# googlegenomics/spark-examples

Measured on NVIDIA H100. Metric: genotype-cells/sec (N x V) into Gram, higher is better.
Workload: dtype int8

## Files before the change

### spark_examples_b200/csrc/gram_sm90.cu

```cuda
#include <cuda.h>
#include <cuda_runtime.h>

#include <cstring>

#include <algorithm>
#include <map>
#include <mutex>
#include <tuple>
#include <type_traits>
#include <cstdio>
#include <cstdlib>
#include <string>
#include <vector>

#include "ptx_sm90.cuh"
#include "vpca_internal.h"

namespace vpca {

namespace {

constexpr int kThreads = 384;
constexpr int kKBytes = 128;
constexpr int kBoxRows = 128;
// ... 22 lines not shown
    int flags;
    int acc_cols;
    int pad1;
};
constexpr int kTileXpose = 1, kTileFiller = 2, kTileSelfB = 4;
constexpr int kMaxSegs = 4;

struct GramArgs {
    int32_t* S;
    int32_t* peer[kMaxPeers];
    int num_peers;
    int peer_mode;
    int own_end[kMaxPeers];
    const TileDesc* tiles;
    int* err;
    int n;
    int num_tiles;
    int num_full;
    int total_weight;
    int kb_total;
    int kb_window;
    int num_workers;
    int resident;
    int kc_per_kb;
    int kb_per_panel;
    int sync_lead;
    int active_workers;
    int* win_done;
    long long* prof;
    const double* cum;
    int col_limit;
    int acc_stride;
    int row_limit;
    int red64;
};

struct Seg {
    int tile, kb0, kb1, col, slot, first, flush, use, win, last_in_win;
    int rowA0, rowA1, rowB, n_eff, flags;
};

struct SegPlan {
    int n;
    int tile[kMaxSegs], lo[kMaxSegs], hi[kMaxSegs], col[kMaxSegs];
    int cols;
    int overflow;
};

__host__ __device__ inline void plan_segments(const TileDesc* tiles, int num_tiles, int first_tile, long long u_begin,
                                              long long u_end, int len, SegPlan& p) {
    p.n = 0;
    p.cols = 0;
    p.overflow = 0;
    const long long origin = (long long)tiles[first_tile].wstart * len;
    long long u = u_begin;
    int t = first_tile;
    while (u < u_end && t < num_tiles) {
        const int w = tiles[t].n_eff >> 4;
        const long long base = (long long)tiles[t].wstart * len - origin;
        const long long tend = base + (long long)w * len;
        if (tend <= u) {
            ++t;
            continue;
        }
        const long long e = u_end < tend ? u_end : tend;
        const int lo = (int)((u - base) / w);
        const int hi = e == tend ? len : (int)((e - base) / w);
// ... 222 lines not shown
        __nanosleep(256);
    }
}

__device__ __forceinline__ uint64_t make_smem_desc(uint32_t saddr) {
    return (uint64_t)((saddr & 0x3FFFFu) >> 4) | (1ull << 16) | ((uint64_t)(1024 >> 4) << 32) | (1ull << 62);
}

__device__ __forceinline__ uint32_t e2m1x4_to_s8x2(uint32_t w) {
    const uint32_t mag = __byte_perm(0x03020100u, 0x0C080604u, w & 0x7777u);
    const uint32_t sgn = ((w >> 3) & 1u) | (((w >> 7) & 1u) << 8) | (((w >> 11) & 1u) << 16) | (((w >> 15) & 1u) << 24);
    const uint32_t m = sgn * 0xFFu;
    return (mag & ~m) | (__vneg4(mag) & m);
}

__device__ __forceinline__ int quarter_rn(int acc) {
    const int q = acc >> 2, r = acc & 3;
    return q + ((r > 2 || (r == 2 && (q & 1))) ? 1 : 0);
}

template <int KIND>
using AccT = typename std::conditional<KIND == 1, float, uint32_t>::type;

template <int KIND>
__device__ __forceinline__ int acc_to_int(AccT<KIND> v) {
    if constexpr (KIND == 0) return (int)v;
    else if constexpr (KIND == 1) return __float2int_rn(v);
    else return quarter_rn((int)v);
}

template <int CG, int KIND>
__global__ void __launch_bounds__(kThreads, 1) gram_kernel(const __grid_constant__ CUtensorMap tmap, const GramArgs a) {
    using C = Cfg<KIND>;
    extern __shared__ uint8_t smem_raw[];
    const uint32_t smem_base = (ptx::smem_u32(smem_raw) + 1023u) & ~1023u;
    const uint32_t bar_base = smem_base + C::STAGES * C::STAGE_BYTES + C::XBUF_BYTES * 2;
    auto sB = [&](uint32_t st) { return smem_base + st * C::STAGE_BYTES; };
    auto sA = [&](uint32_t st) { return smem_base + st * C::STAGE_BYTES + C::B_BYTES; };
    auto full_bar = [&](uint32_t i) { return bar_base + 8u * i; };
    auto empty_bar = [&](uint32_t i) { return bar_base + 8u * (C::STAGES + i); };

    const int warp = __shfl_sync(0xffffffffu, (int)(threadIdx.x >> 5), 0);
    const uint32_t lane = ptx::lane_id();
    const uint32_t cta_rank = (CG == 2) ? (blockIdx.x & 1u) : 0u;
    const int worker = (CG == 2) ? (int)(blockIdx.x >> 1) : (int)blockIdx.x;
    auto release = [&](uint32_t st) {
        if constexpr (CG == 2) {
            ptx::mbar_arrive_cluster(ptx::mapa(empty_bar(st), 0));
            ptx::mbar_arrive_cluster(ptx::mapa(empty_bar(st), 1));
        } else {
            ptx::mbar_arrive(empty_bar(st));
        }
    };

    if (warp == 0 && ptx::elect_one()) {
        ptx::prefetch_tensormap(&tmap);
        for (uint32_t i = 0; i < (uint32_t)C::STAGES; ++i) {
            ptx::mbar_init(full_bar(i), 1);
            ptx::mbar_init(empty_bar(i), 2 * CG);
        }
        ptx::fence_mbar_init();
    }
    if constexpr (CG == 2) ptx::cluster_sync();
    else __syncthreads();
    if (a.prof != nullptr && threadIdx.x == 0) a.prof[(size_t)blockIdx.x * 4 + 0] = globaltimer_ns();

    if (warp < 4) {
        asm volatile("setmaxnreg.dec.sync.aligned.u32 40;");
        if (warp == 0 && ptx::elect_one()) {
            const bool leader = cta_rank == 0;
            Sched sc;
            sc.init(a, worker);
            Seg s;
            uint32_t it = 0;
            int synced_win = -1;
            while (sc.next(s)) {
                const int rowA = (CG == 2 && cta_rank != 0) ? s.rowA1 : s.rowA0;
                const bool two_boxes = s.n_eff > kBoxRows;
                const bool self_b = (CG == 2) && (s.flags & kTileSelfB) != 0;
                const uint32_t tx = (uint32_t)((two_boxes ? 2 : 1) + (self_b ? 0 : 1)) * C::BOX_BYTES;
                if (a.sync_lead > 0 && leader && s.win != synced_win) {
                    synced_win = s.win;
                    if (s.win >= a.sync_lead) wait_window(a.win_done, s.win - a.sync_lead, a.active_workers);
                }
                for (int kb = s.kb0; kb < s.kb1; ++kb, ++it) {
                    const uint32_t st = it % C::STAGES, ph = (it / C::STAGES) & 1u;
                    mbar_wait(empty_bar(st), ph ^ 1u, a.err, 1);
                    const int pnl = kb / a.kb_per_panel;
                    const int kc = (kb - pnl * a.kb_per_panel) * a.kc_per_kb;
                    ptx::mbar_arrive_expect_tx(full_bar(st), tx);
                    if constexpr (CG == 2) {
                        if (two_boxes || cta_rank == 0)
                            ptx::tma_load_3d_multicast(sB(st) + cta_rank * C::BOX_BYTES, &tmap, full_bar(st), kc,
                                                       s.rowB + (int)cta_rank * kBoxRows, pnl, 0x3);
                    } else {
                        ptx::tma_load_3d(sB(st), &tmap, full_bar(st), kc, s.rowB, pnl);
                        if (two_boxes) ptx::tma_load_3d(sB(st) + C::BOX_BYTES, &tmap, full_bar(st), kc, s.rowB + kBoxRows, pnl);
                    }
                    if (!self_b) ptx::tma_load_3d(sA(st), &tmap, full_bar(st), kc, rowA, pnl);
                }
                if (a.sync_lead > 0 && leader && s.last_in_win)
                    asm volatile("red.release.gpu.global.add.s32 [%0], 1;" ::"l"(a.win_done + s.win) : "memory");
            }
        }
    } else {
        asm volatile("setmaxnreg.inc.sync.aligned.u32 232;");
        const int cw = (warp >> 2) - 1;
        const int wq = warp & 3;
        const uint32_t ctid = threadIdx.x - 128;
        AccT<KIND> acc[2][64];
        Sched sc;
        sc.init(a, worker);
        Seg s;
        uint32_t it = 0;
        while (sc.next(s)) {
            const bool filler = (CG == 2) && cta_rank != 0 && (s.flags & kTileFiller) != 0;
            const bool self_b = (CG == 2) && (s.flags & kTileSelfB) != 0;
            const int mrow0 = cw * 128;
            const bool act0 = mrow0 < s.n_eff, act1 = mrow0 + 64 < s.n_eff;
            if (s.first) {
#pragma unroll
                for (int i = 0; i < 64; ++i) {
                    acc[0][i] = 0;
                    acc[1][i] = 0;
                }
            }
            const uint32_t a_off = (self_b ? cta_rank : 2u) * (uint32_t)(kBoxRows * 128);
            int pending = -1;
            for (int kb = s.kb0; kb < s.kb1; ++kb, ++it) {
                const uint32_t st = it % C::STAGES, ph = (it / C::STAGES) & 1u;
                mbar_wait(full_bar(st), ph, a.err, 3);
                uint32_t opB, opA;
                if constexpr (KIND == 2) {
                    const uint32_t xb = smem_base + C::STAGES * C::STAGE_BYTES + (it & 1u) * C::XBUF_BYTES;
                    ptx::named_sync(1, 256);
                    const int nb = s.n_eff > kBoxRows ? 2 * kBoxRows : kBoxRows;
                    const int rows = nb + (self_b ? 0 : kBoxRows);
                    for (int c = (int)ctid; c < rows * 8; c += 256) {
                        const int r = c >> 3, j = c & 7;
                        const uint32_t src = (r < nb ? sB(st) + (uint32_t)r * 64u : sA(st) + (uint32_t)(r - nb) * 64u) + (uint32_t)j * 8u;
                        const int xr = r < nb ? r : 2 * kBoxRows + (r - nb);
                        uint32_t lo, hi;
                        asm volatile("ld.shared.v2.u32 {%0, %1}, [%2];" : "=r"(lo), "=r"(hi) : "r"(src));
                        const uint32_t o0 = e2m1x4_to_s8x2(lo & 0xFFFFu), o1 = e2m1x4_to_s8x2(lo >> 16);
                        const uint32_t o2 = e2m1x4_to_s8x2(hi & 0xFFFFu), o3 = e2m1x4_to_s8x2(hi >> 16);
                        const uint32_t dst = xb + (uint32_t)xr * 128u + (((uint32_t)j ^ ((uint32_t)xr & 7u)) << 4);
                        asm volatile("st.shared.v4.u32 [%0], {%1, %2, %3, %4};" ::"r"(dst), "r"(o0), "r"(o1), "r"(o2), "r"(o3)
                                     : "memory");
                    }
                    ptx::fence_proxy_async();
                    ptx::named_sync(1, 256);
                    if (threadIdx.x % 128 == 0) release(st);
                    opB = xb;
                } else {
                    opB = sB(st);
                }
                opA = opB + a_off;
                const uint64_t bdesc = make_smem_desc(opA);
                const uint64_t adesc0 = make_smem_desc(opB + (uint32_t)mrow0 * 128u);
                const uint64_t adesc1 = make_smem_desc(opB + (uint32_t)(mrow0 + 64) * 128u);
                ptx::wgmma_fence_acc(acc[0]);
                ptx::wgmma_fence_acc(acc[1]);
                ptx::wgmma_fence();
#pragma unroll
                for (int k = 0; k < kKBytes / 32; ++k) {
                    if constexpr (KIND == 1) {
                        ptx::wgmma_bf16(acc[0], adesc0 + 2 * k, bdesc + 2 * k);
                        ptx::wgmma_bf16(acc[1], adesc1 + 2 * k, bdesc + 2 * k);
                    } else {
                        ptx::wgmma_s8(acc[0], adesc0 + 2 * k, bdesc + 2 * k);
                        ptx::wgmma_s8(acc[1], adesc1 + 2 * k, bdesc + 2 * k);
                    }
                }
                ptx::wgmma_commit();
                ptx::wgmma_wait<1>();
                ptx::wgmma_fence_acc(acc[0]);
                ptx::wgmma_fence_acc(acc[1]);
                if constexpr (KIND != 2) {
                    if (pending >= 0 && threadIdx.x % 128 == 0) release((uint32_t)pending);
                }
                pending = (int)st;
            }
            ptx::wgmma_wait<0>();
            ptx::wgmma_fence_acc(acc[0]);
            ptx::wgmma_fence_acc(acc[1]);
            if constexpr (KIND != 2) {
                if (pending >= 0 && threadIdx.x % 128 == 0) release((uint32_t)pending);
            }
            if (!s.flush || filler) continue;

            const int colA = (CG == 2 && cta_rank != 0) ? s.rowA1 : s.rowA0;
            const int row_end = min(a.row_limit, s.rowB + s.n_eff);
            const bool pair64 = a.red64 != 0 && (a.n & 1) == 0;
#pragma unroll
            for (int j = 0; j < 2; ++j) {
                if (!(j == 0 ? act0 : act1)) continue;
#pragma unroll
                for (int h = 0; h < 2; ++h) {
                    const int row = s.rowB + mrow0 + 64 * j + 16 * wq + (int)(lane >> 2) + 8 * h;
                    if (row >= row_end) continue;
                    int32_t* own = a.S;
                    if (a.num_peers != 0 && a.peer_mode == 1) {
                        int o = 0;
                        while (o + 1 < a.num_peers && row >= a.own_end[o]) ++o;
                        own = a.peer[o];
                    }
#pragma unroll
                    for (int i = 0; i < 16; ++i) {
                        const int col = colA + 8 * i + 2 * (int)(lane & 3);
                        if (col >= a.n) continue;
                        int v0 = acc_to_int<KIND>(acc[j][4 * i + 2 * h]);
                        int v1 = acc_to_int<KIND>(acc[j][4 * i + 2 * h + 1]);
                        if ((s.flags & kTileXpose) != 0 && (row >> 7) < (col >> 7)) {
                            for (int e = 0; e < 2; ++e) {
                                const int v = e ? v1 : v0, c = col + e;
                                if (v == 0 || c >= a.n) continue;
                                const size_t o = (size_t)c * (size_t)a.n + (size_t)row;
                                if (a.num_peers == 0) {
                                    asm volatile("red.global.add.s32 [%0], %1;" ::"l"(a.S + o), "r"(v) : "memory");
                                } else if (a.peer_mode == 1) {
                                    int q = 0;
                                    while (q + 1 < a.num_peers && c >= a.own_end[q]) ++q;
                                    asm volatile("red.relaxed.sys.global.add.s32 [%0], %1;" ::"l"(a.peer[q] + o), "r"(v) : "memory");
                                } else {
                                    for (int d = 0; d < a.num_peers; ++d)
                                        asm volatile("red.relaxed.sys.global.add.s32 [%0], %1;" ::"l"(a.peer[d] + o), "r"(v)
                                                     : "memory");
                                }
                            }
                            continue;
                        }
                        if (row < col) v0 = 0;
                        if (row < col + 1 || col + 1 >= a.n) v1 = 0;
                        if ((v0 | v1) == 0) continue;
                        const size_t o = (size_t)row * (size_t)a.n + (size_t)col;
                        if (pair64) {
                            const unsigned long long packed = (unsigned long long)(unsigned)v0 | ((unsigned long long)(unsigned)v1 << 32);
                            if (a.num_peers == 0) {
                                asm volatile("red.global.add.u64 [%0], %1;" ::"l"(a.S + o), "l"(packed) : "memory");
                            } else if (a.peer_mode == 1) {
                                asm volatile("red.relaxed.sys.global.add.u64 [%0], %1;" ::"l"(own + o), "l"(packed) : "memory");
                            } else {
                                for (int d = 0; d < a.num_peers; ++d)
                                    asm volatile("red.relaxed.sys.global.add.u64 [%0], %1;" ::"l"(a.peer[d] + o), "l"(packed)
                                                 : "memory");
                            }
                        } else {
                            for (int e = 0; e < 2; ++e) {
                                const int v = e ? v1 : v0;
                                if (v == 0) continue;
                                if (a.num_peers == 0) {
                                    asm volatile("red.global.add.s32 [%0], %1;" ::"l"(a.S + o + e), "r"(v) : "memory");
                                } else if (a.peer_mode == 1) {
                                    asm volatile("red.relaxed.sys.global.add.s32 [%0], %1;" ::"l"(own + o + e), "r"(v) : "memory");
                                } else {
                                    for (int d = 0; d < a.num_peers; ++d)
                                        asm volatile("red.relaxed.sys.global.add.s32 [%0], %1;" ::"l"(a.peer[d] + o + e), "r"(v)
                                                     : "memory");
                                }
                            }
                        }
                    }
                }
            }
        }
        if (a.prof != nullptr && threadIdx.x == 128) a.prof[(size_t)blockIdx.x * 4 + 2] = globaltimer_ns();
    }

    if constexpr (CG == 2) ptx::cluster_sync();
    else __syncthreads();
    if (a.prof != nullptr && threadIdx.x == 0) a.prof[(size_t)blockIdx.x * 4 + 3] = globaltimer_ns();
}

__global__ void rebalance_kernel(const long long* __restrict__ prof, double* __restrict__ cum, int workers, int cta_group,
                                 double gain, double max_share, long long min_ns, int* __restrict__ gen, const TileDesc* __restrict__ tiles,
                                 int num_tiles, int total_weight, int kbw, int col_limit) {
    __shared__ double sh[1024];
    __shared__ double cand[1025];
    __shared__ long long need[1025];
    __shared__ double red_sum, red_min;
    __shared__ int reject, need_repair;
    const int w = threadIdx.x;
    const bool active = w < workers;
    double t = 0.0, share_old = 0.0;
    if (active) {
        const long long t0 = prof[(size_t)w * cta_group * 4 + 0], t1 = prof[(size_t)w * cta_group * 4 + 2];
        t = (double)(t1 - t0);
        share_old = cum[w + 1] - cum[w];
    }
    sh[w] = active ? t : 1e30;
    if (w == 0) {
        reject = 0;
        need_repair = 0;
// ... 460 lines not shown
        for (int i = 0; i < p.n; ++i, ++cnt)
            if (cnt < max_pieces) {
                int32_t* o = out + (size_t)cnt * 6;
                o[0] = w; o[1] = p.tile[i]; o[2] = p.lo[i]; o[3] = p.hi[i]; o[4] = p.col[i]; o[5] = p.cols;
            }
    }
    return cnt;
}

cudaError_t gram_accumulate(GramPlan& plan, const void* d_x, int elem_bits, int n, int64_t nv, int64_t ld, int64_t panel,
                            int32_t* d_S, cudaStream_t stream, std::string* err) {
    if (nv <= 0) return cudaSuccess;
    EncodeTiledFn encode = get_encode_fn();
    if (encode == nullptr) {
        if (err) *err = "cuTensorMapEncodeTiled entry point not available";
        return cudaErrorNotSupported;
    }
    if (plan.num_sms == 0) {
        int dev = 0;
        cudaGetDevice(&dev);
        cudaDeviceGetAttribute(&plan.num_sms, cudaDevAttrMultiProcessorCount, dev);
        const char* cg = getenv("VPCA_CTA_GROUP");
        if (cg != nullptr) plan.cta_group = (atoi(cg) == 1) ? 1 : 2;
        const char* kw = getenv("VPCA_KB_WINDOW");
        if (kw != nullptr) plan.kb_window = atoi(kw);
        const char* sl = getenv("VPCA_SYNC_LEAD");
        if (sl != nullptr) plan.sync_lead = atoi(sl);
        const char* pf = getenv("VPCA_GRAM_PROF");
        plan.profile = (pf != nullptr && atoi(pf) != 0);
        const char* ad = getenv("VPCA_ADAPTIVE");
        if (ad != nullptr) plan.adaptive = atoi(ad) != 0;
        const char* sb = getenv("VPCA_SELF_B");
        if (sb != nullptr) plan.self_b = atoi(sb) != 0;
        const char* r64 = getenv("VPCA_RED64");
        if (r64 != nullptr) plan.red64 = atoi(r64) != 0;
        const char* gain = getenv("VPCA_REBALANCE_GAIN");
        if (gain != nullptr) plan.gain = std::min(1.0, std::max(0.1, atof(gain)));
        const char* ex = getenv("VPCA_EXACT_COVER");
        if (ex != nullptr) plan.exact_cover = atoi(ex) != 0;
    }
    if (plan.d_win_done == nullptr) {
        cudaError_t e = cudaMalloc(&plan.d_win_done, GramPlan::kMaxWindows * sizeof(int));
        if (e != cudaSuccess) return e;
    }
    if ((plan.profile || plan.adaptive) && plan.d_prof == nullptr) {
        cudaError_t e = cudaMalloc(&plan.d_prof, 1024 * 4 * sizeof(long long));
        if (e != cudaSuccess) return e;
        e = cudaMemsetAsync(plan.d_prof, 0, 1024 * 4 * sizeof(long long), stream);
        if (e != cudaSuccess) return e;
    }
    if (plan.d_err == nullptr) {
        cudaError_t e = cudaHostAlloc(&plan.d_err, 4 * sizeof(int), cudaHostAllocMapped);
        if (e != cudaSuccess) return e;
        for (int i = 0; i < 4; ++i) plan.d_err[i] = 0;
    }
    const int tile_bn = kUmmaN;
    const bool banded = plan.own_hi > plan.own_lo && plan.num_peers <= 1;
    const int row_lo = banded ? plan.own_lo : 0, row_hi = banded ? plan.own_hi : n;
    const bool exact = plan.exact_cover && !banded;
    if (plan.tiles_for_n != n || plan.tiles_for_cg != plan.cta_group || plan.tiles_for_bn != (exact ? -1 : tile_bn) ||
        plan.tiles_row_lo != row_lo || plan.tiles_row_hi != row_hi) {
        cudaError_t e = build_tiles(plan, n, exact, tile_bn, row_lo, row_hi, stream);
        if (e != cudaSuccess) return e;
    }
    if (panel > 0) {
        if ((panel % 128) != 0) {
            if (err) *err = "panel_variants must be a multiple of 128";
            return cudaErrorInvalidValue;
// ... 30 lines not shown
                                   (cuuint64_t)n * (cuuint64_t)ld * (cuuint64_t)elem_bits / 8};
    const int kc_per_kb = elem_bits == 4 ? elems_per_kb / 2 : elems_per_kb;
    const cuuint32_t box[3] = {(cuuint32_t)kc_per_kb, (cuuint32_t)kBoxRows, 1};
    const cuuint32_t estr[3] = {1, 1, 1};
    const CUtensorMapDataType tmtype = elem_bits == 16 ? CU_TENSOR_MAP_DATA_TYPE_BFLOAT16 : CU_TENSOR_MAP_DATA_TYPE_UINT8;
    CUresult r = encode(&tmap, tmtype, 3,
                        const_cast<void*>(d_x), gdim, gstride, box, estr, CU_TENSOR_MAP_INTERLEAVE_NONE,
                        elem_bits == 4 ? CU_TENSOR_MAP_SWIZZLE_NONE : CU_TENSOR_MAP_SWIZZLE_128B,
                        CU_TENSOR_MAP_L2_PROMOTION_L2_256B, CU_TENSOR_MAP_FLOAT_OOB_FILL_NONE);
    if (r != CUDA_SUCCESS) {
        if (err) *err = "cuTensorMapEncodeTiled failed with CUresult " + std::to_string((int)r);
        return cudaErrorInvalidValue;
    }

    GramArgs args{};
    args.S = banded ? d_S - (ptrdiff_t)plan.own_lo * n : d_S;
    args.num_peers = (plan.num_peers > 1 && d_S == plan.peer_base[plan.peer_rank]) ? plan.num_peers : 0;
    for (int d = 0; d < kMaxPeers; ++d) args.peer[d] = d < plan.num_peers ? plan.peer_S[d] : nullptr;
    args.peer_mode = plan.peer_mode;
    for (int d = 0; d < kMaxPeers; ++d) args.own_end[d] = plan.own_end[d];
    args.tiles = static_cast<const TileDesc*>(plan.d_tiles);
    cudaHostGetDevicePointer(reinterpret_cast<void**>(&args.err), plan.d_err, 0);
    args.n = n;
    args.num_tiles = plan.num_tiles;
    args.num_full = plan.num_full;
    args.total_weight = plan.total_weight;
    args.kb_total = (int)((nv + elems_per_kb - 1) / elems_per_kb);
    args.kb_per_panel = panel > 0 ? (int)(panel / elems_per_kb) : args.kb_total;
    args.num_workers = workers;
    args.kc_per_kb = kc_per_kb;
    args.acc_stride = 0;
    args.col_limit = plan.tiles_col_limit;
    args.row_limit = row_hi;
    args.red64 = plan.red64 ? 1 : 0;
    {
        int kbw = plan.kb_window;
        if (kbw <= 0 && panel > 0) kbw = args.kb_per_panel;
        if (kbw <= 0) {
            const long long target = 16ll << 20;
            kbw = (int)std::max<long long>(8, std::min<long long>(4096, target / ((long long)n * kKBytes)));
        }
        kbw = std::min(kbw, args.kb_total);
        std::vector<double> cum0;
        args.resident = (plan.num_tiles <= 4 * workers && initial_split(plan, workers, kbw, cum0)) ? 1 : 0;
        int dev = 0;
        cudaGetDevice(&dev);
        args.kb_window = args.resident ? kbw : args.kb_total;
        if (args.resident && (plan.d_cum == nullptr || plan.cum_workers != workers || plan.cum_tiles != plan.num_tiles ||
                              plan.cum_kbw != kbw || plan.cum_for_n != n || plan.cum_elem != elem_bits)) {
            remember_split(plan);
            if (plan.adaptive && !banded) {
                std::lock_guard<std::mutex> lk(g_split_mu);
                auto it = g_splits.find(SplitKey{dev, n, plan.num_tiles, kbw, workers, elem_bits});
                if (it != g_splits.end()) {
                    std::vector<double> learned = it->second;
                    const TileDesc* tiles = reinterpret_cast<const TileDesc*>(plan.h_tiles.data());
                    std::vector<long long> need((size_t)workers + 1);
                    if (repair_split(tiles, plan.num_tiles, workers, (long long)plan.total_weight * kbw, kbw, plan.tiles_col_limit,
                                     learned.data(), need.data()))
                        cum0 = learned;
                }
            }
            if (plan.d_cum) cudaFree(plan.d_cum);
            plan.d_cum = nullptr;
            cudaError_t e = cudaMalloc(&plan.d_cum, (size_t)(workers + 2) * sizeof(double) + sizeof(int));
            if (e != cudaSuccess) return e;
            cum0.push_back(0.0);
// ... 128 lines not shown
```

### spark_examples_b200/csrc/ptx_sm90.cuh

```cuda
#pragma once
#include <cstdint>
#include <cuda_runtime.h>

namespace vpca {
namespace ptx {

__device__ __forceinline__ uint32_t smem_u32(const void* p) {
    return static_cast<uint32_t>(__cvta_generic_to_shared(p));
}

__device__ __forceinline__ uint32_t lane_id() {
    uint32_t r;
    asm volatile("mov.u32 %0, %%laneid;" : "=r"(r));
    return r;
}

__device__ __forceinline__ bool elect_one() {
    uint32_t pred = 0;
    asm volatile(
        "{\n\t"
        ".reg .pred P;\n\t"
        "elect.sync _|P, 0xffffffff;\n\t"
        "selp.u32 %0, 1, 0, P;\n\t"
        "}\n"
// ... 60 lines not shown
    asm volatile("barrier.cluster.arrive.release;\n\tbarrier.cluster.wait.acquire;" ::: "memory");
}
__device__ __forceinline__ void wgmma_fence() { asm volatile("wgmma.fence.sync.aligned;" ::: "memory"); }
__device__ __forceinline__ void wgmma_commit() { asm volatile("wgmma.commit_group.sync.aligned;" ::: "memory"); }
template <int N>
__device__ __forceinline__ void wgmma_wait() { asm volatile("wgmma.wait_group.sync.aligned %0;" ::"n"(N) : "memory"); }
__device__ __forceinline__ void wgmma_fence_acc(uint32_t (&d)[64]) {
#pragma unroll
    for (int i = 0; i < 64; ++i) asm volatile("" : "+r"(d[i])::"memory");
}
__device__ __forceinline__ void wgmma_fence_acc(float (&d)[64]) {
#pragma unroll
    for (int i = 0; i < 64; ++i) asm volatile("" : "+f"(d[i])::"memory");
}

__device__ __forceinline__ void wgmma_s8(uint32_t (&d)[64], uint64_t a_desc, uint64_t b_desc) {
    asm volatile(
        "{\n\t.reg .pred p;\n\tsetp.ne.b32 p, 1, 0;\n\t"
        "wgmma.mma_async.sync.aligned.m64n128k32.s32.s8.s8 "
        "{%0, %1, %2, %3, %4, %5, %6, %7, %8, %9, %10, %11, %12, %13, %14, %15, %16, %17, %18, %19, %20, %21, %22, %23, %24, %25, %26, %27, %28, %29, %30, %31, %32, %33, %34, %35, %36, %37, %38, %39, %40, %41, %42, %43, %44, %45, %46, %47, %48, %49, %50, %51, %52, %53, %54, %55, %56, %57, %58, %59, %60, %61, %62, %63}, %64, %65, p;\n\t}\n"
        : "+r"(d[0]), "+r"(d[1]), "+r"(d[2]), "+r"(d[3]), "+r"(d[4]), "+r"(d[5]), "+r"(d[6]), "+r"(d[7]), "+r"(d[8]), "+r"(d[9]), "+r"(d[10]), "+r"(d[11]), "+r"(d[12]), "+r"(d[13]), "+r"(d[14]), "+r"(d[15]), "+r"(d[16]), "+r"(d[17]), "+r"(d[18]), "+r"(d[19]), "+r"(d[20]), "+r"(d[21]), "+r"(d[22]), "+r"(d[23]), "+r"(d[24]), "+r"(d[25]), "+r"(d[26]), "+r"(d[27]), "+r"(d[28]), "+r"(d[29]), "+r"(d[30]), "+r"(d[31]), "+r"(d[32]), "+r"(d[33]), "+r"(d[34]), "+r"(d[35]), "+r"(d[36]), "+r"(d[37]), "+r"(d[38]), "+r"(d[39]), "+r"(d[40]), "+r"(d[41]), "+r"(d[42]), "+r"(d[43]), "+r"(d[44]), "+r"(d[45]), "+r"(d[46]), "+r"(d[47]), "+r"(d[48]), "+r"(d[49]), "+r"(d[50]), "+r"(d[51]), "+r"(d[52]), "+r"(d[53]), "+r"(d[54]), "+r"(d[55]), "+r"(d[56]), "+r"(d[57]), "+r"(d[58]), "+r"(d[59]), "+r"(d[60]), "+r"(d[61]), "+r"(d[62]), "+r"(d[63])
        : "l"(a_desc), "l"(b_desc));
}

__device__ __forceinline__ void wgmma_bf16(float (&f)[64], uint64_t a_desc, uint64_t b_desc) {
    asm volatile(
        "{\n\t.reg .pred p;\n\tsetp.ne.b32 p, 1, 0;\n\t"
        "wgmma.mma_async.sync.aligned.m64n128k16.f32.bf16.bf16 "
        "{%0, %1, %2, %3, %4, %5, %6, %7, %8, %9, %10, %11, %12, %13, %14, %15, %16, %17, %18, %19, %20, %21, %22, %23, %24, %25, %26, %27, %28, %29, %30, %31, %32, %33, %34, %35, %36, %37, %38, %39, %40, %41, %42, %43, %44, %45, %46, %47, %48, %49, %50, %51, %52, %53, %54, %55, %56, %57, %58, %59, %60, %61, %62, %63}, %64, %65, p, 1, 1, 0, 0;\n\t}\n"
        : "+f"(f[0]), "+f"(f[1]), "+f"(f[2]), "+f"(f[3]), "+f"(f[4]), "+f"(f[5]), "+f"(f[6]), "+f"(f[7]), "+f"(f[8]), "+f"(f[9]), "+f"(f[10]), "+f"(f[11]), "+f"(f[12]), "+f"(f[13]), "+f"(f[14]), "+f"(f[15]), "+f"(f[16]), "+f"(f[17]), "+f"(f[18]), "+f"(f[19]), "+f"(f[20]), "+f"(f[21]), "+f"(f[22]), "+f"(f[23]), "+f"(f[24]), "+f"(f[25]), "+f"(f[26]), "+f"(f[27]), "+f"(f[28]), "+f"(f[29]), "+f"(f[30]), "+f"(f[31]), "+f"(f[32]), "+f"(f[33]), "+f"(f[34]), "+f"(f[35]), "+f"(f[36]), "+f"(f[37]), "+f"(f[38]), "+f"(f[39]), "+f"(f[40]), "+f"(f[41]), "+f"(f[42]), "+f"(f[43]), "+f"(f[44]), "+f"(f[45]), "+f"(f[46]), "+f"(f[47]), "+f"(f[48]), "+f"(f[49]), "+f"(f[50]), "+f"(f[51]), "+f"(f[52]), "+f"(f[53]), "+f"(f[54]), "+f"(f[55]), "+f"(f[56]), "+f"(f[57]), "+f"(f[58]), "+f"(f[59]), "+f"(f[60]), "+f"(f[61]), "+f"(f[62]), "+f"(f[63])
        : "l"(a_desc), "l"(b_desc));
}

__device__ __forceinline__ void named_sync(uint32_t id, uint32_t count) {
    asm volatile("bar.sync %0, %1;" ::"r"(id), "r"(count) : "memory");
}

}
}
```

### spark_examples_b200/csrc/vpca_internal.h

```cpp
#pragma once
#include <cstdint>
#include <cuda_runtime.h>
#include <string>
#include <vector>

#include "../../include/vpca.h"

namespace vpca {

struct GramPlan {
    int cta_group = 2;
    int kb_window = 0;
    int num_sms = 0;
    int max_pairs[3] = {};
    void* d_tiles = nullptr;
    std::vector<int32_t> h_tiles;
    int num_tiles = 0;
    int num_full = 0;
    int total_weight = 0;
    int tiles_col_limit = 256;
    bool exact_cover = false;
    int tiles_for_n = -1;
    int tiles_for_cg = 0;
    int tiles_for_bn = 0;
    int tiles_row_lo = 0, tiles_row_hi = 0;
    int own_lo = 0, own_hi = 0;
    int last_resident = 0;
    int* d_err = nullptr;
    static constexpr int kMaxWindows = 1 << 16;
    int sync_lead = 0;
    int* d_win_done = nullptr;
    bool self_b = true;
    bool red64 = true;
    double gain = 0.5;
    bool adaptive = true;
    double* d_cum = nullptr;
    int cum_workers = 0, cum_tiles = 0, cum_kbw = 0, cum_for_n = 0, cum_dev = 0, cum_elem = 0;
    int num_peers = 0, peer_rank = 0, peer_epoch = 0;
    int32_t* peer_S[16] = {};
    int32_t* peer_base[16] = {};
    int32_t* peer_flags[16] = {};
    int band_row0[16] = {}, band_rows[16] = {};
    bool peers_ipc = false;
    int peer_mode = 0;
    int own_end[16] = {};
    bool profile = false;
    long long* d_prof = nullptr;
};
int gram_read_profile(GramPlan& plan, long long* out, int max_ctas);

cudaError_t gram_accumulate(GramPlan& plan, const void* d_x, int elem_bits, int n, int64_t nv, int64_t ld, int64_t panel,
                            int32_t* d_S, cudaStream_t stream, std::string* err);
cudaError_t gram_symmetrize(int32_t* d_S, int n, cudaStream_t stream);
cudaError_t gram_add(int32_t* d_dst, const int32_t* d_src, int64_t count, cudaStream_t stream);
cudaError_t gram_add_peers(GramPlan& plan, const int32_t* d_src, int64_t count, cudaStream_t stream);
cudaError_t gram_add_owners(GramPlan& plan, const int32_t* d_src, int n, cudaStream_t stream);
cudaError_t gram_gather_rows(GramPlan& plan, int32_t* d_S, int n, cudaStream_t stream);
cudaError_t gram_peer_barrier(GramPlan& plan, cudaStream_t stream);
cudaError_t gram_preload_kernels(cudaStream_t stream);
cudaError_t encode_preload_kernels();
void gram_plan_free(GramPlan& plan);
int gram_debug_max_clusters(int cluster_size);
int gram_debug_band_tiles(int n, int cta_group, int row_lo, int row_hi, int32_t* out, int max_tiles);
int gram_debug_tiles(int n, int cta_group, int exact, int32_t* out, int max_tiles);
int gram_debug_plan(const int32_t* tiles8, int num_tiles, int workers, int kbw, int32_t* out, int max_pieces);
int gram_debug_repair(const int32_t* tiles8, int num_tiles, int workers, int kbw, int col_limit, double* cum, int32_t* out,
// ... 152 lines not shown
```

Before: 534.4 billion.

## Use m64n256 WGMMA with multicast A tiles for 2-CTA cluster path

For the 2-CTA cluster configuration (non-FP4 kinds), each CTA now loads its own 128-row B slice and both A boxes arrive by multicast. Each consumer warpgroup then issues a single m64n256 WGMMA covering both A column blocks instead of two m64n128 instructions. Flush logic is remapped so the second accumulator writes to rowA1 columns. This halves WGMMA issue count and raises per-instruction N, improving operand reuse. The cost is a changed shared-memory layout and filler-tile handling, plus reliance on a multicast of A that must match the cluster scheduling.

```diff
diff --git a/spark_examples_b200/csrc/gram_sm90.cu b/spark_examples_b200/csrc/gram_sm90.cu
--- a/spark_examples_b200/csrc/gram_sm90.cu
+++ b/spark_examples_b200/csrc/gram_sm90.cu
@@ -367,11 +367,13 @@
 template <int CG, int KIND>
 __global__ void __launch_bounds__(kThreads, 1) gram_kernel(const __grid_constant__ CUtensorMap tmap, const GramArgs a) {
     using C = Cfg<KIND>;
+    constexpr bool WIDE = CG == 2 && KIND != 2;
+    constexpr uint32_t kBBytes = WIDE ? C::BOX_BYTES : C::B_BYTES;
     extern __shared__ uint8_t smem_raw[];
     const uint32_t smem_base = (ptx::smem_u32(smem_raw) + 1023u) & ~1023u;
     const uint32_t bar_base = smem_base + C::STAGES * C::STAGE_BYTES + C::XBUF_BYTES * 2;
     auto sB = [&](uint32_t st) { return smem_base + st * C::STAGE_BYTES; };
-    auto sA = [&](uint32_t st) { return smem_base + st * C::STAGE_BYTES + C::B_BYTES; };
+    auto sA = [&](uint32_t st) { return smem_base + st * C::STAGE_BYTES + kBBytes; };
     auto full_bar = [&](uint32_t i) { return bar_base + 8u * i; };
     auto empty_bar = [&](uint32_t i) { return bar_base + 8u * (C::STAGES + i); };
 
@@ -423,6 +425,13 @@
                     mbar_wait(empty_bar(st), ph ^ 1u, a.err, 1);
                     const int pnl = kb / a.kb_per_panel;
                     const int kc = (kb - pnl * a.kb_per_panel) * a.kc_per_kb;
+                    if constexpr (WIDE) {
+                        ptx::mbar_arrive_expect_tx(full_bar(st), (uint32_t)(self_b ? 2 : 3) * C::BOX_BYTES);
+                        if (!self_b)
+                            ptx::tma_load_3d(sB(st), &tmap, full_bar(st), kc, s.rowB + (int)cta_rank * kBoxRows, pnl);
+                        ptx::tma_load_3d_multicast(sA(st) + cta_rank * C::BOX_BYTES, &tmap, full_bar(st), kc, rowA, pnl, 0x3);
+                        continue;
+                    }
                     ptx::mbar_arrive_expect_tx(full_bar(st), tx);
                     if constexpr (CG == 2) {
                         if (two_boxes || cta_rank == 0)
@@ -449,10 +458,10 @@
         Seg s;
         uint32_t it = 0;
         while (sc.next(s)) {
-            const bool filler = (CG == 2) && cta_rank != 0 && (s.flags & kTileFiller) != 0;
+            const bool filler = (CG == 2) && (WIDE || cta_rank != 0) && (s.flags & kTileFiller) != 0;
             const bool self_b = (CG == 2) && (s.flags & kTileSelfB) != 0;
-            const int mrow0 = cw * 128;
-            const bool act0 = mrow0 < s.n_eff, act1 = mrow0 + 64 < s.n_eff;
+            const int mrow0 = WIDE ? (int)cta_rank * 128 + cw * 64 : cw * 128;
+            const bool act0 = mrow0 < s.n_eff, act1 = WIDE ? act0 && !filler : mrow0 + 64 < s.n_eff;
             if (s.first) {
 #pragma unroll
                 for (int i = 0; i < 64; ++i) {
@@ -491,15 +500,24 @@
                     opB = sB(st);
                 }
                 opA = opB + a_off;
+                if constexpr (WIDE) {
+                    opA = sA(st);
+                    opB = self_b ? opA + cta_rank * (uint32_t)C::BOX_BYTES : sB(st);
+                }
                 const uint64_t bdesc = make_smem_desc(opA);
                 const uint64_t adesc0 = make_smem_desc(opB + (uint32_t)mrow0 * 128u);
                 const uint64_t adesc1 = make_smem_desc(opB + (uint32_t)(mrow0 + 64) * 128u);
+                const uint64_t adescw = make_smem_desc(opB + (uint32_t)(cw * 64) * 128u);
                 ptx::wgmma_fence_acc(acc[0]);
                 ptx::wgmma_fence_acc(acc[1]);
                 ptx::wgmma_fence();
 #pragma unroll
                 for (int k = 0; k < kKBytes / 32; ++k) {
-                    if constexpr (KIND == 1) {
+                    if constexpr (WIDE && KIND == 1) {
+                        ptx::wgmma_bf16_n256(acc[0], acc[1], adescw + 2 * k, bdesc + 2 * k);
+                    } else if constexpr (WIDE) {
+                        ptx::wgmma_s8_n256(acc[0], acc[1], adescw + 2 * k, bdesc + 2 * k);
+                    } else if constexpr (KIND == 1) {
                         ptx::wgmma_bf16(acc[0], adesc0 + 2 * k, bdesc + 2 * k);
                         ptx::wgmma_bf16(acc[1], adesc1 + 2 * k, bdesc + 2 * k);
                     } else {
@@ -522,9 +540,9 @@
             if constexpr (KIND != 2) {
                 if (pending >= 0 && threadIdx.x % 128 == 0) release((uint32_t)pending);
             }
-            if (!s.flush || filler) continue;
-
-            const int colA = (CG == 2 && cta_rank != 0) ? s.rowA1 : s.rowA0;
+            if (!s.flush || (filler && !WIDE)) continue;
+
+            const int colA = (CG == 2 && cta_rank != 0 && !WIDE) ? s.rowA1 : s.rowA0;
             const int row_end = min(a.row_limit, s.rowB + s.n_eff);
             const bool pair64 = a.red64 != 0 && (a.n & 1) == 0;
 #pragma unroll
@@ -532,7 +550,7 @@
                 if (!(j == 0 ? act0 : act1)) continue;
 #pragma unroll
                 for (int h = 0; h < 2; ++h) {
-                    const int row = s.rowB + mrow0 + 64 * j + 16 * wq + (int)(lane >> 2) + 8 * h;
+                    const int row = s.rowB + mrow0 + (WIDE ? 0 : 64 * j) + 16 * wq + (int)(lane >> 2) + 8 * h;
                     if (row >= row_end) continue;
                     int32_t* own = a.S;
                     if (a.num_peers != 0 && a.peer_mode == 1) {
@@ -542,7 +560,7 @@
                     }
 #pragma unroll
                     for (int i = 0; i < 16; ++i) {
-                        const int col = colA + 8 * i + 2 * (int)(lane & 3);
+                        const int col = (WIDE && j == 1 ? s.rowA1 : colA) + 8 * i + 2 * (int)(lane & 3);
                         if (col >= a.n) continue;
                         int v0 = acc_to_int<KIND>(acc[j][4 * i + 2 * h]);
                         int v1 = acc_to_int<KIND>(acc[j][4 * i + 2 * h + 1]);
diff --git a/spark_examples_b200/csrc/ptx_sm90.cuh b/spark_examples_b200/csrc/ptx_sm90.cuh
--- a/spark_examples_b200/csrc/ptx_sm90.cuh
+++ b/spark_examples_b200/csrc/ptx_sm90.cuh
@@ -116,6 +116,24 @@
         : "l"(a_desc), "l"(b_desc));
 }
 
+__device__ __forceinline__ void wgmma_s8_n256(uint32_t (&d0)[64], uint32_t (&d1)[64], uint64_t a_desc, uint64_t b_desc) {
+    asm volatile(
+        "{\n\t.reg .pred p;\n\tsetp.ne.b32 p, 1, 0;\n\t"
+        "wgmma.mma_async.sync.aligned.m64n256k32.s32.s8.s8 "
+        "{%0, %1, %2, %3, %4, %5, %6, %7, %8, %9, %10, %11, %12, %13, %14, %15, %16, %17, %18, %19, %20, %21, %22, %23, %24, %25, %26, %27, %28, %29, %30, %31, %32, %33, %34, %35, %36, %37, %38, %39, %40, %41, %42, %43, %44, %45, %46, %47, %48, %49, %50, %51, %52, %53, %54, %55, %56, %57, %58, %59, %60, %61, %62, %63, %64, %65, %66, %67, %68, %69, %70, %71, %72, %73, %74, %75, %76, %77, %78, %79, %80, %81, %82, %83, %84, %85, %86, %87, %88, %89, %90, %91, %92, %93, %94, %95, %96, %97, %98, %99, %100, %101, %102, %103, %104, %105, %106, %107, %108, %109, %110, %111, %112, %113, %114, %115, %116, %117, %118, %119, %120, %121, %122, %123, %124, %125, %126, %127}, %128, %129, p;\n\t}\n"
+        : "+r"(d0[0]), "+r"(d0[1]), "+r"(d0[2]), "+r"(d0[3]), "+r"(d0[4]), "+r"(d0[5]), "+r"(d0[6]), "+r"(d0[7]), "+r"(d0[8]), "+r"(d0[9]), "+r"(d0[10]), "+r"(d0[11]), "+r"(d0[12]), "+r"(d0[13]), "+r"(d0[14]), "+r"(d0[15]), "+r"(d0[16]), "+r"(d0[17]), "+r"(d0[18]), "+r"(d0[19]), "+r"(d0[20]), "+r"(d0[21]), "+r"(d0[22]), "+r"(d0[23]), "+r"(d0[24]), "+r"(d0[25]), "+r"(d0[26]), "+r"(d0[27]), "+r"(d0[28]), "+r"(d0[29]), "+r"(d0[30]), "+r"(d0[31]), "+r"(d0[32]), "+r"(d0[33]), "+r"(d0[34]), "+r"(d0[35]), "+r"(d0[36]), "+r"(d0[37]), "+r"(d0[38]), "+r"(d0[39]), "+r"(d0[40]), "+r"(d0[41]), "+r"(d0[42]), "+r"(d0[43]), "+r"(d0[44]), "+r"(d0[45]), "+r"(d0[46]), "+r"(d0[47]), "+r"(d0[48]), "+r"(d0[49]), "+r"(d0[50]), "+r"(d0[51]), "+r"(d0[52]), "+r"(d0[53]), "+r"(d0[54]), "+r"(d0[55]), "+r"(d0[56]), "+r"(d0[57]), "+r"(d0[58]), "+r"(d0[59]), "+r"(d0[60]), "+r"(d0[61]), "+r"(d0[62]), "+r"(d0[63]), "+r"(d1[0]), "+r"(d1[1]), "+r"(d1[2]), "+r"(d1[3]), "+r"(d1[4]), "+r"(d1[5]), "+r"(d1[6]), "+r"(d1[7]), "+r"(d1[8]), "+r"(d1[9]), "+r"(d1[10]), "+r"(d1[11]), "+r"(d1[12]), "+r"(d1[13]), "+r"(d1[14]), "+r"(d1[15]), "+r"(d1[16]), "+r"(d1[17]), "+r"(d1[18]), "+r"(d1[19]), "+r"(d1[20]), "+r"(d1[21]), "+r"(d1[22]), "+r"(d1[23]), "+r"(d1[24]), "+r"(d1[25]), "+r"(d1[26]), "+r"(d1[27]), "+r"(d1[28]), "+r"(d1[29]), "+r"(d1[30]), "+r"(d1[31]), "+r"(d1[32]), "+r"(d1[33]), "+r"(d1[34]), "+r"(d1[35]), "+r"(d1[36]), "+r"(d1[37]), "+r"(d1[38]), "+r"(d1[39]), "+r"(d1[40]), "+r"(d1[41]), "+r"(d1[42]), "+r"(d1[43]), "+r"(d1[44]), "+r"(d1[45]), "+r"(d1[46]), "+r"(d1[47]), "+r"(d1[48]), "+r"(d1[49]), "+r"(d1[50]), "+r"(d1[51]), "+r"(d1[52]), "+r"(d1[53]), "+r"(d1[54]), "+r"(d1[55]), "+r"(d1[56]), "+r"(d1[57]), "+r"(d1[58]), "+r"(d1[59]), "+r"(d1[60]), "+r"(d1[61]), "+r"(d1[62]), "+r"(d1[63])
+        : "l"(a_desc), "l"(b_desc));
+}
+
+__device__ __forceinline__ void wgmma_bf16_n256(float (&d0)[64], float (&d1)[64], uint64_t a_desc, uint64_t b_desc) {
+    asm volatile(
+        "{\n\t.reg .pred p;\n\tsetp.ne.b32 p, 1, 0;\n\t"
+        "wgmma.mma_async.sync.aligned.m64n256k16.f32.bf16.bf16 "
+        "{%0, %1, %2, %3, %4, %5, %6, %7, %8, %9, %10, %11, %12, %13, %14, %15, %16, %17, %18, %19, %20, %21, %22, %23, %24, %25, %26, %27, %28, %29, %30, %31, %32, %33, %34, %35, %36, %37, %38, %39, %40, %41, %42, %43, %44, %45, %46, %47, %48, %49, %50, %51, %52, %53, %54, %55, %56, %57, %58, %59, %60, %61, %62, %63, %64, %65, %66, %67, %68, %69, %70, %71, %72, %73, %74, %75, %76, %77, %78, %79, %80, %81, %82, %83, %84, %85, %86, %87, %88, %89, %90, %91, %92, %93, %94, %95, %96, %97, %98, %99, %100, %101, %102, %103, %104, %105, %106, %107, %108, %109, %110, %111, %112, %113, %114, %115, %116, %117, %118, %119, %120, %121, %122, %123, %124, %125, %126, %127}, %128, %129, p, 1, 1, 0, 0;\n\t}\n"
+        : "+f"(d0[0]), "+f"(d0[1]), "+f"(d0[2]), "+f"(d0[3]), "+f"(d0[4]), "+f"(d0[5]), "+f"(d0[6]), "+f"(d0[7]), "+f"(d0[8]), "+f"(d0[9]), "+f"(d0[10]), "+f"(d0[11]), "+f"(d0[12]), "+f"(d0[13]), "+f"(d0[14]), "+f"(d0[15]), "+f"(d0[16]), "+f"(d0[17]), "+f"(d0[18]), "+f"(d0[19]), "+f"(d0[20]), "+f"(d0[21]), "+f"(d0[22]), "+f"(d0[23]), "+f"(d0[24]), "+f"(d0[25]), "+f"(d0[26]), "+f"(d0[27]), "+f"(d0[28]), "+f"(d0[29]), "+f"(d0[30]), "+f"(d0[31]), "+f"(d0[32]), "+f"(d0[33]), "+f"(d0[34]), "+f"(d0[35]), "+f"(d0[36]), "+f"(d0[37]), "+f"(d0[38]), "+f"(d0[39]), "+f"(d0[40]), "+f"(d0[41]), "+f"(d0[42]), "+f"(d0[43]), "+f"(d0[44]), "+f"(d0[45]), "+f"(d0[46]), "+f"(d0[47]), "+f"(d0[48]), "+f"(d0[49]), "+f"(d0[50]), "+f"(d0[51]), "+f"(d0[52]), "+f"(d0[53]), "+f"(d0[54]), "+f"(d0[55]), "+f"(d0[56]), "+f"(d0[57]), "+f"(d0[58]), "+f"(d0[59]), "+f"(d0[60]), "+f"(d0[61]), "+f"(d0[62]), "+f"(d0[63]), "+f"(d1[0]), "+f"(d1[1]), "+f"(d1[2]), "+f"(d1[3]), "+f"(d1[4]), "+f"(d1[5]), "+f"(d1[6]), "+f"(d1[7]), "+f"(d1[8]), "+f"(d1[9]), "+f"(d1[10]), "+f"(d1[11]), "+f"(d1[12]), "+f"(d1[13]), "+f"(d1[14]), "+f"(d1[15]), "+f"(d1[16]), "+f"(d1[17]), "+f"(d1[18]), "+f"(d1[19]), "+f"(d1[20]), "+f"(d1[21]), "+f"(d1[22]), "+f"(d1[23]), "+f"(d1[24]), "+f"(d1[25]), "+f"(d1[26]), "+f"(d1[27]), "+f"(d1[28]), "+f"(d1[29]), "+f"(d1[30]), "+f"(d1[31]), "+f"(d1[32]), "+f"(d1[33]), "+f"(d1[34]), "+f"(d1[35]), "+f"(d1[36]), "+f"(d1[37]), "+f"(d1[38]), "+f"(d1[39]), "+f"(d1[40]), "+f"(d1[41]), "+f"(d1[42]), "+f"(d1[43]), "+f"(d1[44]), "+f"(d1[45]), "+f"(d1[46]), "+f"(d1[47]), "+f"(d1[48]), "+f"(d1[49]), "+f"(d1[50]), "+f"(d1[51]), "+f"(d1[52]), "+f"(d1[53]), "+f"(d1[54]), "+f"(d1[55]), "+f"(d1[56]), "+f"(d1[57]), "+f"(d1[58]), "+f"(d1[59]), "+f"(d1[60]), "+f"(d1[61]), "+f"(d1[62]), "+f"(d1[63])
+        : "l"(a_desc), "l"(b_desc));
+}
+
 __device__ __forceinline__ void named_sync(uint32_t id, uint32_t count) {
     asm volatile("bar.sync %0, %1;" ::"r"(id), "r"(count) : "memory");
 }
```

New measurement: 544.7 billion (median of 6 runs). 1.9% higher.

## Switch consumer MMA to m64n256 wgmma with transposed operand roles and epilogue

Applied to the files above, without the earlier changes.

Each consumer warpgroup now issues a single m64n256 wgmma per k-step, using 64 rows of the A box as M and the full 256-row B block as N. This replaces two m64n128 wgmmas that shared the same B descriptor, and is meant to cut shared-memory operand traffic and the number of wgmma issues. The epilogue is rewritten for the transposed accumulator layout, and the packed 64-bit red64 atomic path and its env knob are removed. The cost is that every nonzero value now needs its own 32-bit atomic, and the N=256 tile is always computed even when n_eff covers only one box.

```diff
diff --git a/spark_examples_b200/csrc/gram_sm90.cu b/spark_examples_b200/csrc/gram_sm90.cu
--- a/spark_examples_b200/csrc/gram_sm90.cu
+++ b/spark_examples_b200/csrc/gram_sm90.cu
@@ -78,7 +78,6 @@
     int col_limit;
     int acc_stride;
     int row_limit;
-    int red64;
 };
 
 struct Seg {
@@ -443,7 +442,7 @@
         const int cw = (warp >> 2) - 1;
         const int wq = warp & 3;
         const uint32_t ctid = threadIdx.x - 128;
-        AccT<KIND> acc[2][64];
+        AccT<KIND> acc[128];
         Sched sc;
         sc.init(a, worker);
         Seg s;
@@ -451,14 +450,9 @@
         while (sc.next(s)) {
             const bool filler = (CG == 2) && cta_rank != 0 && (s.flags & kTileFiller) != 0;
             const bool self_b = (CG == 2) && (s.flags & kTileSelfB) != 0;
-            const int mrow0 = cw * 128;
-            const bool act0 = mrow0 < s.n_eff, act1 = mrow0 + 64 < s.n_eff;
             if (s.first) {
 #pragma unroll
-                for (int i = 0; i < 64; ++i) {
-                    acc[0][i] = 0;
-                    acc[1][i] = 0;
-                }
+                for (int i = 0; i < 128; ++i) acc[i] = 0;
             }
             const uint32_t a_off = (self_b ? cta_rank : 2u) * (uint32_t)(kBoxRows * 128);
             int pending = -1;
@@ -491,34 +485,25 @@
                     opB = sB(st);
                 }
                 opA = opB + a_off;
-                const uint64_t bdesc = make_smem_desc(opA);
-                const uint64_t adesc0 = make_smem_desc(opB + (uint32_t)mrow0 * 128u);
-                const uint64_t adesc1 = make_smem_desc(opB + (uint32_t)(mrow0 + 64) * 128u);
-                ptx::wgmma_fence_acc(acc[0]);
-                ptx::wgmma_fence_acc(acc[1]);
+                const uint64_t mdesc = make_smem_desc(opA + (uint32_t)(64 * cw) * 128u);
+                const uint64_t ndesc = make_smem_desc(opB);
+                ptx::wgmma_fence_acc(acc);
                 ptx::wgmma_fence();
 #pragma unroll
                 for (int k = 0; k < kKBytes / 32; ++k) {
-                    if constexpr (KIND == 1) {
-                        ptx::wgmma_bf16(acc[0], adesc0 + 2 * k, bdesc + 2 * k);
-                        ptx::wgmma_bf16(acc[1], adesc1 + 2 * k, bdesc + 2 * k);
-                    } else {
-                        ptx::wgmma_s8(acc[0], adesc0 + 2 * k, bdesc + 2 * k);
-                        ptx::wgmma_s8(acc[1], adesc1 + 2 * k, bdesc + 2 * k);
-                    }
+                    if constexpr (KIND == 1) ptx::wgmma_bf16_n256(acc, mdesc + 2 * k, ndesc + 2 * k);
+                    else ptx::wgmma_s8_n256(acc, mdesc + 2 * k, ndesc + 2 * k);
                 }
                 ptx::wgmma_commit();
                 ptx::wgmma_wait<1>();
-                ptx::wgmma_fence_acc(acc[0]);
-                ptx::wgmma_fence_acc(acc[1]);
+                ptx::wgmma_fence_acc(acc);
                 if constexpr (KIND != 2) {
                     if (pending >= 0 && threadIdx.x % 128 == 0) release((uint32_t)pending);
                 }
                 pending = (int)st;
             }
             ptx::wgmma_wait<0>();
-            ptx::wgmma_fence_acc(acc[0]);
-            ptx::wgmma_fence_acc(acc[1]);
+            ptx::wgmma_fence_acc(acc);
             if constexpr (KIND != 2) {
                 if (pending >= 0 && threadIdx.x % 128 == 0) release((uint32_t)pending);
             }
@@ -526,74 +511,35 @@
 
             const int colA = (CG == 2 && cta_rank != 0) ? s.rowA1 : s.rowA0;
             const int row_end = min(a.row_limit, s.rowB + s.n_eff);
-            const bool pair64 = a.red64 != 0 && (a.n & 1) == 0;
 #pragma unroll
-            for (int j = 0; j < 2; ++j) {
-                if (!(j == 0 ? act0 : act1)) continue;
+            for (int h = 0; h < 2; ++h) {
+                const int col = colA + 64 * cw + 16 * wq + (int)(lane >> 2) + 8 * h;
+                if (col >= a.n) continue;
 #pragma unroll
-                for (int h = 0; h < 2; ++h) {
-                    const int row = s.rowB + mrow0 + 64 * j + 16 * wq + (int)(lane >> 2) + 8 * h;
-                    if (row >= row_end) continue;
-                    int32_t* own = a.S;
-                    if (a.num_peers != 0 && a.peer_mode == 1) {
-                        int o = 0;
-                        while (o + 1 < a.num_peers && row >= a.own_end[o]) ++o;
-                        own = a.peer[o];
-                    }
+                for (int i = 0; i < 32; ++i) {
 #pragma unroll
-                    for (int i = 0; i < 16; ++i) {
-                        const int col = colA + 8 * i + 2 * (int)(lane & 3);
-                        if (col >= a.n) continue;
-                        int v0 = acc_to_int<KIND>(acc[j][4 * i + 2 * h]);
-                        int v1 = acc_to_int<KIND>(acc[j][4 * i + 2 * h + 1]);
+                    for (int e = 0; e < 2; ++e) {
+                        const int row = s.rowB + 8 * i + 2 * (int)(lane & 3) + e;
+                        if (row >= row_end) continue;
+                        const int v = acc_to_int<KIND>(acc[4 * i + 2 * h + e]);
+                        if (v == 0) continue;
+                        int r = row, c = col;
                         if ((s.flags & kTileXpose) != 0 && (row >> 7) < (col >> 7)) {
-                            for (int e = 0; e < 2; ++e) {
-                                const int v = e ? v1 : v0, c = col + e;
-                                if (v == 0 || c >= a.n) continue;
-                                const size_t o = (size_t)c * (size_t)a.n + (size_t)row;
-                                if (a.num_peers == 0) {
-                                    asm volatile("red.global.add.s32 [%0], %1;" ::"l"(a.S + o), "r"(v) : "memory");
-                                } else if (a.peer_mode == 1) {
-                                    int q = 0;
-                                    while (q + 1 < a.num_peers && c >= a.own_end[q]) ++q;
-                                    asm volatile("red.relaxed.sys.global.add.s32 [%0], %1;" ::"l"(a.peer[q] + o), "r"(v) : "memory");
-                                } else {
-                                    for (int d = 0; d < a.num_peers; ++d)
-                                        asm volatile("red.relaxed.sys.global.add.s32 [%0], %1;" ::"l"(a.peer[d] + o), "r"(v)
-                                                     : "memory");
-                                }
-                            }
+                            r = col;
+                            c = row;
+                        } else if (row < col) {
                             continue;
                         }
-                        if (row < col) v0 = 0;
-                        if (row < col + 1 || col + 1 >= a.n) v1 = 0;
-                        if ((v0 | v1) == 0) continue;
-                        const size_t o = (size_t)row * (size_t)a.n + (size_t)col;
-                        if (pair64) {
-                            const unsigned long long packed = (unsigned long long)(unsigned)v0 | ((unsigned long long)(unsigned)v1 << 32);
-                            if (a.num_peers == 0) {
-                                asm volatile("red.global.add.u64 [%0], %1;" ::"l"(a.S + o), "l"(packed) : "memory");
-                            } else if (a.peer_mode == 1) {
-                                asm volatile("red.relaxed.sys.global.add.u64 [%0], %1;" ::"l"(own + o), "l"(packed) : "memory");
-                            } else {
-                                for (int d = 0; d < a.num_peers; ++d)
-                                    asm volatile("red.relaxed.sys.global.add.u64 [%0], %1;" ::"l"(a.peer[d] + o), "l"(packed)
-                                                 : "memory");
-                            }
+                        const size_t o = (size_t)r * (size_t)a.n + (size_t)c;
+                        if (a.num_peers == 0) {
+                            asm volatile("red.global.add.s32 [%0], %1;" ::"l"(a.S + o), "r"(v) : "memory");
+                        } else if (a.peer_mode == 1) {
+                            int q = 0;
+                            while (q + 1 < a.num_peers && r >= a.own_end[q]) ++q;
+                            asm volatile("red.relaxed.sys.global.add.s32 [%0], %1;" ::"l"(a.peer[q] + o), "r"(v) : "memory");
                         } else {
-                            for (int e = 0; e < 2; ++e) {
-                                const int v = e ? v1 : v0;
-                                if (v == 0) continue;
-                                if (a.num_peers == 0) {
-                                    asm volatile("red.global.add.s32 [%0], %1;" ::"l"(a.S + o + e), "r"(v) : "memory");
-                                } else if (a.peer_mode == 1) {
-                                    asm volatile("red.relaxed.sys.global.add.s32 [%0], %1;" ::"l"(own + o + e), "r"(v) : "memory");
-                                } else {
-                                    for (int d = 0; d < a.num_peers; ++d)
-                                        asm volatile("red.relaxed.sys.global.add.s32 [%0], %1;" ::"l"(a.peer[d] + o + e), "r"(v)
-                                                     : "memory");
-                                }
-                            }
+                            for (int d = 0; d < a.num_peers; ++d)
+                                asm volatile("red.relaxed.sys.global.add.s32 [%0], %1;" ::"l"(a.peer[d] + o), "r"(v) : "memory");
                         }
                     }
                 }
@@ -1120,8 +1066,6 @@
         if (ad != nullptr) plan.adaptive = atoi(ad) != 0;
         const char* sb = getenv("VPCA_SELF_B");
         if (sb != nullptr) plan.self_b = atoi(sb) != 0;
-        const char* r64 = getenv("VPCA_RED64");
-        if (r64 != nullptr) plan.red64 = atoi(r64) != 0;
         const char* gain = getenv("VPCA_REBALANCE_GAIN");
         if (gain != nullptr) plan.gain = std::min(1.0, std::max(0.1, atof(gain)));
         const char* ex = getenv("VPCA_EXACT_COVER");
@@ -1218,7 +1162,6 @@
     args.acc_stride = 0;
     args.col_limit = plan.tiles_col_limit;
     args.row_limit = row_hi;
-    args.red64 = plan.red64 ? 1 : 0;
     {
         int kbw = plan.kb_window;
         if (kbw <= 0 && panel > 0) kbw = args.kb_per_panel;
diff --git a/spark_examples_b200/csrc/ptx_sm90.cuh b/spark_examples_b200/csrc/ptx_sm90.cuh
--- a/spark_examples_b200/csrc/ptx_sm90.cuh
+++ b/spark_examples_b200/csrc/ptx_sm90.cuh
@@ -116,6 +116,33 @@
         : "l"(a_desc), "l"(b_desc));
 }
 
+__device__ __forceinline__ void wgmma_fence_acc(uint32_t (&d)[128]) {
+#pragma unroll
+    for (int i = 0; i < 128; ++i) asm volatile("" : "+r"(d[i])::"memory");
+}
+__device__ __forceinline__ void wgmma_fence_acc(float (&d)[128]) {
+#pragma unroll
+    for (int i = 0; i < 128; ++i) asm volatile("" : "+f"(d[i])::"memory");
+}
+
+__device__ __forceinline__ void wgmma_s8_n256(uint32_t (&d)[128], uint64_t a_desc, uint64_t b_desc) {
+    asm volatile(
+        "{\n\t.reg .pred p;\n\tsetp.ne.b32 p, 1, 0;\n\t"
+        "wgmma.mma_async.sync.aligned.m64n256k32.s32.s8.s8 "
+        "{%0, %1, %2, %3, %4, %5, %6, %7, %8, %9, %10, %11, %12, %13, %14, %15, %16, %17, %18, %19, %20, %21, %22, %23, %24, %25, %26, %27, %28, %29, %30, %31, %32, %33, %34, %35, %36, %37, %38, %39, %40, %41, %42, %43, %44, %45, %46, %47, %48, %49, %50, %51, %52, %53, %54, %55, %56, %57, %58, %59, %60, %61, %62, %63, %64, %65, %66, %67, %68, %69, %70, %71, %72, %73, %74, %75, %76, %77, %78, %79, %80, %81, %82, %83, %84, %85, %86, %87, %88, %89, %90, %91, %92, %93, %94, %95, %96, %97, %98, %99, %100, %101, %102, %103, %104, %105, %106, %107, %108, %109, %110, %111, %112, %113, %114, %115, %116, %117, %118, %119, %120, %121, %122, %123, %124, %125, %126, %127}, %128, %129, p;\n\t}\n"
+        : "+r"(d[0]), "+r"(d[1]), "+r"(d[2]), "+r"(d[3]), "+r"(d[4]), "+r"(d[5]), "+r"(d[6]), "+r"(d[7]), "+r"(d[8]), "+r"(d[9]), "+r"(d[10]), "+r"(d[11]), "+r"(d[12]), "+r"(d[13]), "+r"(d[14]), "+r"(d[15]), "+r"(d[16]), "+r"(d[17]), "+r"(d[18]), "+r"(d[19]), "+r"(d[20]), "+r"(d[21]), "+r"(d[22]), "+r"(d[23]), "+r"(d[24]), "+r"(d[25]), "+r"(d[26]), "+r"(d[27]), "+r"(d[28]), "+r"(d[29]), "+r"(d[30]), "+r"(d[31]), "+r"(d[32]), "+r"(d[33]), "+r"(d[34]), "+r"(d[35]), "+r"(d[36]), "+r"(d[37]), "+r"(d[38]), "+r"(d[39]), "+r"(d[40]), "+r"(d[41]), "+r"(d[42]), "+r"(d[43]), "+r"(d[44]), "+r"(d[45]), "+r"(d[46]), "+r"(d[47]), "+r"(d[48]), "+r"(d[49]), "+r"(d[50]), "+r"(d[51]), "+r"(d[52]), "+r"(d[53]), "+r"(d[54]), "+r"(d[55]), "+r"(d[56]), "+r"(d[57]), "+r"(d[58]), "+r"(d[59]), "+r"(d[60]), "+r"(d[61]), "+r"(d[62]), "+r"(d[63]), "+r"(d[64]), "+r"(d[65]), "+r"(d[66]), "+r"(d[67]), "+r"(d[68]), "+r"(d[69]), "+r"(d[70]), "+r"(d[71]), "+r"(d[72]), "+r"(d[73]), "+r"(d[74]), "+r"(d[75]), "+r"(d[76]), "+r"(d[77]), "+r"(d[78]), "+r"(d[79]), "+r"(d[80]), "+r"(d[81]), "+r"(d[82]), "+r"(d[83]), "+r"(d[84]), "+r"(d[85]), "+r"(d[86]), "+r"(d[87]), "+r"(d[88]), "+r"(d[89]), "+r"(d[90]), "+r"(d[91]), "+r"(d[92]), "+r"(d[93]), "+r"(d[94]), "+r"(d[95]), "+r"(d[96]), "+r"(d[97]), "+r"(d[98]), "+r"(d[99]), "+r"(d[100]), "+r"(d[101]), "+r"(d[102]), "+r"(d[103]), "+r"(d[104]), "+r"(d[105]), "+r"(d[106]), "+r"(d[107]), "+r"(d[108]), "+r"(d[109]), "+r"(d[110]), "+r"(d[111]), "+r"(d[112]), "+r"(d[113]), "+r"(d[114]), "+r"(d[115]), "+r"(d[116]), "+r"(d[117]), "+r"(d[118]), "+r"(d[119]), "+r"(d[120]), "+r"(d[121]), "+r"(d[122]), "+r"(d[123]), "+r"(d[124]), "+r"(d[125]), "+r"(d[126]), "+r"(d[127])
+        : "l"(a_desc), "l"(b_desc));
+}
+
+__device__ __forceinline__ void wgmma_bf16_n256(float (&d)[128], uint64_t a_desc, uint64_t b_desc) {
+    asm volatile(
+        "{\n\t.reg .pred p;\n\tsetp.ne.b32 p, 1, 0;\n\t"
+        "wgmma.mma_async.sync.aligned.m64n256k16.f32.bf16.bf16 "
+        "{%0, %1, %2, %3, %4, %5, %6, %7, %8, %9, %10, %11, %12, %13, %14, %15, %16, %17, %18, %19, %20, %21, %22, %23, %24, %25, %26, %27, %28, %29, %30, %31, %32, %33, %34, %35, %36, %37, %38, %39, %40, %41, %42, %43, %44, %45, %46, %47, %48, %49, %50, %51, %52, %53, %54, %55, %56, %57, %58, %59, %60, %61, %62, %63, %64, %65, %66, %67, %68, %69, %70, %71, %72, %73, %74, %75, %76, %77, %78, %79, %80, %81, %82, %83, %84, %85, %86, %87, %88, %89, %90, %91, %92, %93, %94, %95, %96, %97, %98, %99, %100, %101, %102, %103, %104, %105, %106, %107, %108, %109, %110, %111, %112, %113, %114, %115, %116, %117, %118, %119, %120, %121, %122, %123, %124, %125, %126, %127}, %128, %129, p, 1, 1, 0, 0;\n\t}\n"
+        : "+f"(d[0]), "+f"(d[1]), "+f"(d[2]), "+f"(d[3]), "+f"(d[4]), "+f"(d[5]), "+f"(d[6]), "+f"(d[7]), "+f"(d[8]), "+f"(d[9]), "+f"(d[10]), "+f"(d[11]), "+f"(d[12]), "+f"(d[13]), "+f"(d[14]), "+f"(d[15]), "+f"(d[16]), "+f"(d[17]), "+f"(d[18]), "+f"(d[19]), "+f"(d[20]), "+f"(d[21]), "+f"(d[22]), "+f"(d[23]), "+f"(d[24]), "+f"(d[25]), "+f"(d[26]), "+f"(d[27]), "+f"(d[28]), "+f"(d[29]), "+f"(d[30]), "+f"(d[31]), "+f"(d[32]), "+f"(d[33]), "+f"(d[34]), "+f"(d[35]), "+f"(d[36]), "+f"(d[37]), "+f"(d[38]), "+f"(d[39]), "+f"(d[40]), "+f"(d[41]), "+f"(d[42]), "+f"(d[43]), "+f"(d[44]), "+f"(d[45]), "+f"(d[46]), "+f"(d[47]), "+f"(d[48]), "+f"(d[49]), "+f"(d[50]), "+f"(d[51]), "+f"(d[52]), "+f"(d[53]), "+f"(d[54]), "+f"(d[55]), "+f"(d[56]), "+f"(d[57]), "+f"(d[58]), "+f"(d[59]), "+f"(d[60]), "+f"(d[61]), "+f"(d[62]), "+f"(d[63]), "+f"(d[64]), "+f"(d[65]), "+f"(d[66]), "+f"(d[67]), "+f"(d[68]), "+f"(d[69]), "+f"(d[70]), "+f"(d[71]), "+f"(d[72]), "+f"(d[73]), "+f"(d[74]), "+f"(d[75]), "+f"(d[76]), "+f"(d[77]), "+f"(d[78]), "+f"(d[79]), "+f"(d[80]), "+f"(d[81]), "+f"(d[82]), "+f"(d[83]), "+f"(d[84]), "+f"(d[85]), "+f"(d[86]), "+f"(d[87]), "+f"(d[88]), "+f"(d[89]), "+f"(d[90]), "+f"(d[91]), "+f"(d[92]), "+f"(d[93]), "+f"(d[94]), "+f"(d[95]), "+f"(d[96]), "+f"(d[97]), "+f"(d[98]), "+f"(d[99]), "+f"(d[100]), "+f"(d[101]), "+f"(d[102]), "+f"(d[103]), "+f"(d[104]), "+f"(d[105]), "+f"(d[106]), "+f"(d[107]), "+f"(d[108]), "+f"(d[109]), "+f"(d[110]), "+f"(d[111]), "+f"(d[112]), "+f"(d[113]), "+f"(d[114]), "+f"(d[115]), "+f"(d[116]), "+f"(d[117]), "+f"(d[118]), "+f"(d[119]), "+f"(d[120]), "+f"(d[121]), "+f"(d[122]), "+f"(d[123]), "+f"(d[124]), "+f"(d[125]), "+f"(d[126]), "+f"(d[127])
+        : "l"(a_desc), "l"(b_desc));
+}
+
 __device__ __forceinline__ void named_sync(uint32_t id, uint32_t count) {
     asm volatile("bar.sync %0, %1;" ::"r"(id), "r"(count) : "memory");
 }
diff --git a/spark_examples_b200/csrc/vpca_internal.h b/spark_examples_b200/csrc/vpca_internal.h
--- a/spark_examples_b200/csrc/vpca_internal.h
+++ b/spark_examples_b200/csrc/vpca_internal.h
@@ -31,7 +31,6 @@
     int sync_lead = 0;
     int* d_win_done = nullptr;
     bool self_b = true;
-    bool red64 = true;
     double gain = 0.5;
     bool adaptive = true;
     double* d_cum = nullptr;
```

Measured after the change: 533.9 billion before, 540.0 billion after, median of 6. +1.1%, better.
